# edenartlab/sd-lora-trainer

Hardware: AMD Instinct MI355X
Metric: training images/sec, SDXL 1024px rank-16 LoRA, 1/2/4/8 GPU (job-parallel) (higher is better)
Workload: dtype bf16

## Files before the change

include/sdlt_kernels.h:

```cpp
#ifndef SDLT_KERNELS_H
#define SDLT_KERNELS_H
#include <stdint.h>
#ifdef __cplusplus
extern "C" {
#endif

const char* sdlt_last_error(void);
int sdlt_abi_version(void);
int sdlt_struct_size(int which);

typedef struct sdlt_gemm_batch_item {
  const void* X; const void* W;
  const void* Adown; const void* Bup; void* T_out;
  void* C; void* Ct;
  const float* bias;
  const float* col_scale;
} sdlt_gemm_batch_item;

typedef struct sdlt_gemm_params {
  const void* X; int64_t ldx;
  const void* W; int64_t ldw;
  int32_t M, N, K;
  const void* X2; int64_t ldx2;
  const void* W2; int64_t ldw2;
// ... 411 lines not shown
  float* norm;
  uint8_t* out;
  int32_t n_img, T, P, gh, gw, H, W;
  float alpha;
} sdlt_heatmap_overlay_params;
int sdlt_heatmap_overlay(const sdlt_heatmap_overlay_params* p, void* stream);

int sdlt_token_pool(const void* x, int64_t ldx, int32_t B, int32_t H, int32_t W, int32_t C, const float* gamma, const float* beta, float eps,
                    int32_t f, int32_t mode, void* y, int64_t ldy, int32_t Nkp, void* stream);

int sdlt_tile_blend(const float* tile, int64_t ld, int32_t th, int32_t tw, int32_t C, const float* wy, const float* wx,
                    float* out, int32_t H, int32_t W, int32_t y0, int32_t x0, void* stream);

typedef struct {
  const int32_t* ys; const int32_t* xs;
  const float* wy; const float* wx;
  int32_t n, H, W, th, tw, ty, tx, pad_;
} sdlt_window_params;
int sdlt_window_gather(const sdlt_window_params* p, const void* x_full, void* x_tiles, int64_t ld, const float* tf_full, float* tf_tiles, void* stream);
int sdlt_window_blend(const sdlt_window_params* p, const float* eps_tiles, float* eps_full, void* stream);

int sdlt_add2d(const void* a, int64_t lda, const void* b, int64_t ldb, void* out, int64_t ldo, int32_t M, int32_t C, void* stream);

int sdlt_embed_gather(const void* table, int64_t ld_table, const int64_t* ids, const void* pos, int64_t ld_pos,
                      int32_t B, int32_t T, int32_t Tp, int32_t D, void* out, int64_t ldo, void* stream);
int sdlt_embed_grad(const void* dx, int64_t lddx, const int64_t* ids, const int64_t* train_ids, int32_t n_train,
                    int32_t B, int32_t T, int32_t Tp, int32_t D, float* grad, int32_t accumulate, void* stream);
int sdlt_ti_std_reg(const float* rows, int32_t n, int32_t D, float target_mean, float target_var, float weight,
                    float* grad, float* loss_out, void* stream);

typedef struct sdlt_strip_params {
  const void* X; int64_t ldx;
  const void* W; int64_t ldw;
  const float* bias;
  const void* R; int64_t ldr;
  void* Y; int64_t ldy;
  void* Y2; int64_t ldy2;
  const void* Z; int64_t ldz;
  const float* c1; const float* c2;
  float* stats;
  int32_t B, T, Tp, N, K, act, ln;
  float eps;
  int32_t splitk, cnt_len;
  void* ws; int64_t ws_bytes;
  int32_t* cnt;
  float* P; int64_t ldp;
} sdlt_strip_params;
int sdlt_strip_gemm(const sdlt_strip_params* p, void* stream);

int sdlt_strip_gemm_pair(const sdlt_strip_params* a, const sdlt_strip_params* b, void* stream);
int sdlt_attn_pair_ok(const sdlt_attn_params* a, const sdlt_attn_params* b);
int sdlt_attn_fwd_pair(const sdlt_attn_params* a, const sdlt_attn_params* b, void* stream);
int sdlt_attn_bwd_pair(const sdlt_attn_params* a, const sdlt_attn_params* b, void* stream);
typedef struct sdlt_ln_slabs_params {
  const void* x; int64_t ldx;
  const float* dy32; int64_t lddy32;
  const float* gamma; const float* stats;
  const void* dres; int64_t lddres;
  void* dx; int64_t lddx;
  int32_t nslab, M, C, pad_;
} sdlt_ln_slabs_params;
int sdlt_layernorm_bwd_slabs_pair(const sdlt_ln_slabs_params* a, const sdlt_ln_slabs_params* b, void* stream);

int sdlt_wsk_gemm(const void* X, int64_t ldx, const void* W, int64_t ldw, int32_t M, int32_t N, int32_t K, const float* bias,
                  const void* R, int64_t ldr, void* Y, int64_t ldy, const void* Adown, int64_t ld_adown, const void* Bup, int64_t ld_bup,
                  float lora_scale, void* T_out, int64_t ld_t, int32_t lora_group_k, void* stream);

int sdlt_wsk_gemm_rowdot(const void* X, int64_t ldx, const void* W, int64_t ldw, int32_t M, int32_t N, int32_t K, const float* bias,
                         const void* O, int64_t ldo, void* Y, int64_t ldy, const void* Adown, int64_t ld_adown, const void* Bup, int64_t ld_bup,
                         float lora_scale, void* T_out, int64_t ld_t, int32_t lora_group_k, float* D, int32_t Nq, void* stream);

int sdlt_wsk_pack_weight(const void* W, int64_t ldw, int32_t N, int32_t K, void* Wp, void* stream);

int sdlt_wsk_conv(const void* X, int64_t ldx, const void* W, int64_t ldw, int32_t B, int32_t H, int32_t Wd, int32_t Cin, int32_t N, int32_t flip,
                  const float* bias, const void* rowbias, int64_t ld_rowbias, const void* R, int64_t ldr, void* Y, int64_t ldy,
                  const void* Adown, int64_t ld_adown, const void* Bup, int64_t ld_bup, float lora_scale, void* T_out, int64_t ld_t,
                  const void* zero, void* stream);

int sdlt_wsk_gemm_ln(const void* X, int64_t ldx, const void* W, int64_t ldw, int32_t M, int32_t N, int32_t K, const float* c2,
                     const void* R, int64_t ldr, void* Y, int64_t ldy, const void* Adown, int64_t ld_adown, const void* Bup, int64_t ld_bup,
                     float lora_scale, void* T_out, int64_t ld_t, const float* ln_c1, float* ln_stats, float ln_eps,
                     const float* ln_adapter, void* stream);

typedef struct sdlt_wsk_gemm_params {
  const void* X; int64_t ldx;
  const void* W; int64_t ldw;
  const float* bias;
  const void* R; int64_t ldr;
  void* Y; int64_t ldy;
  const void* Adown; int64_t ld_adown;
  const void* Bup; int64_t ld_bup;
  void* T_out; int64_t ld_t;
  const float* col_scale;
  void* Y0; int64_t ldy0;
  const float* ln_c1; float* ln_stats; const float* ln_adapter;
  void* ln_parts;
  float* dotD;
  const void* pf_next_w;
  int32_t M, N, K;
  int32_t lora_group_k, lora_rp, dot_nq;
  float lora_scale, ln_eps;
  int32_t pf_next_n, pf_next_k, pf_steps, pad_;
} sdlt_wsk_gemm_params;
int sdlt_wsk_gemm_p(const sdlt_wsk_gemm_params* p, void* stream);

int sdlt_wsk_gemm_parts(const void* X, int64_t ldx, const void* W, int64_t ldw, int32_t M, int32_t N, int32_t K, const float* bias,
// ... 28 lines not shown
```

sd-lora-trainer_amd/_lib.py:

```python
import ctypes as C
import os

import torch

_HERE = os.path.dirname(os.path.abspath(__file__))
LIB_PATH = os.environ.get("SDLT_KERNEL_LIB") or os.path.join(_HERE, "libsdlt_kernels.so")

i32, i64, f32, vp = C.c_int32, C.c_int64, C.c_float, C.c_void_p


class GemmParams(C.Structure):
    _fields_ = [
        ("X", vp), ("ldx", i64), ("W", vp), ("ldw", i64),
        ("M", i32), ("N", i32), ("K", i32),
        ("X2", vp), ("ldx2", i64), ("W2", vp), ("ldw2", i64),
        ("K2", i32), ("mode", i32),
        ("Hin", i32), ("Win", i32), ("Cin", i32), ("Hout", i32), ("Wout", i32),
        ("stride", i32), ("ups", i32), ("flip", i32), ("tr", i32),
        ("zero", vp),
        ("Adown", vp), ("ld_adown", i64), ("Bup", vp), ("ld_bup", i64),
        ("T_out", vp), ("ld_t", i64),
        ("lora_R", i32), ("lora_scale", f32), ("alpha", f32),
        ("bias", vp),
        ("rowbias", vp), ("ld_rowbias", i64), ("rows_per_batch", i32),
# ... 222 lines not shown
    "sdlt_groupnorm_fwd": (i32, [C.POINTER(GroupNormParams), vp]),
    "sdlt_groupnorm_bwd": (i32, [C.POINTER(GroupNormParams), vp]),
    "sdlt_layernorm_fwd": (i32, [vp, i64, i32, i32, vp, vp, f32, vp, i64, vp, vp]),
    "sdlt_layernorm_bwd": (i32, [vp, i64, vp, i64, i32, i32, vp, vp, vp, i64, vp, i64, vp]),
    "sdlt_layernorm_bwd_y": (i32, [vp, i64, vp, i64, i32, i32, vp, vp, vp, vp, i64, vp, i64, vp, i64, vp]),
    "sdlt_ln_fold_adapters": (i32, [vp, i32, vp]),
    "sdlt_layernorm_bwd_slabs": (i32, [vp, i64, vp, i64, i32, i32, i32, vp, vp, vp, i64, vp, i64, vp]),
    "sdlt_geglu_fwd": (i32, [vp, i64, i32, i32, vp, i64, vp]),
    "sdlt_geglu_bwd": (i32, [vp, i64, vp, i64, i32, i32, vp, i64, vp]),
    "sdlt_map_bf16": (i32, [i32, vp, vp, vp, i64, vp]),
    "sdlt_timestep_embedding": (i32, [vp, i32, i32, vp, i64, vp]),
    "sdlt_add_noise_nhwc": (i32, [vp, vp, vp, vp, i32, i32, i32, i32, vp, vp, vp]),
    "sdlt_masked_mse_fwd_bwd": (i32, [vp, i64, vp, vp, vp, vp, vp, i32, i32, i32, i32, f32, i32, f32, vp, i32, vp, vp, vp]),
    "sdlt_adamw_fused": (i32, [vp, vp, vp, vp, i64, vp, vp, vp]),
    "sdlt_prodigy_step": (i32, [vp, vp, vp, vp, vp, vp, i64, vp, vp, vp, vp, vp]),
    "sdlt_wgrad_transpose": (i32, [vp, i64, i32, i32, vp, i64, i32, vp, vp]),
    "sdlt_wgrad_im2col_t": (i32, [vp, i64, i32, i32, i32, i32, i32, i32, vp, i64, i32, vp]),
    "sdlt_wgrad_transpose_batch": (i32, [vp, i32, i64, i32, i32, i64, i32, vp]),
    "sdlt_affine_grad_batch": (i32, [vp, i32, i32, i64, i32, i64, i64, i32, i32, i32, f32, i32, vp]),
    "sdlt_wgrad_im2col_t_batch": (i32, [vp, i32, i64, i32, i32, i32, i32, i32, i32, i64, i32, vp]),
    "sdlt_layernorm_affine_grad": (i32, [vp, i64, vp, i64, i32, i32, vp, vp, vp, i32, vp]),
    "sdlt_groupnorm_affine_grad": (i32, [vp, vp, vp, i32, vp]),
    "sdlt_lora_shadow_refresh": (i32, [vp, vp, vp, i32, vp, vp]),
    "sdlt_adamw_shadow_refresh": (i32, [vp, vp, vp, i32, vp, vp, vp, vp, vp, vp]),
    "sdlt_adamw8_shadow_refresh": (i32, [vp, vp, vp, i32, vp, vp, vp, vp, vp, vp, vp, vp]),
    "sdlt_adamw8_flat": (i32, [vp, vp, vp, vp, vp, i64, vp, vp, vp]),
    "sdlt_dora_refresh": (i32, [vp, vp, vp, i32, i32, i32, vp]),
    "sdlt_dora_scale_wt": (i32, [vp, vp, vp, i32, vp]),
    "sdlt_dora_mag_grad": (i32, [vp, vp, vp, i32, vp, vp, i32, vp, vp]),
    "sdlt_lora_merge": (i32, [vp, vp, vp, i32, i32, i32, vp]),
    "sdlt_delta_matmul": (i32, [vp, vp, vp, i32, i32, vp]),
    "sdlt_sampler_step": (i32, [C.POINTER(SamplerParams), vp]),
    "sdlt_sampler_step_img": (i32, [C.POINTER(SamplerImgParams), vp]),
    "sdlt_sampler_step_ms": (i32, [C.POINTER(SamplerMsParams), vp]),
    "sdlt_sampler_step_sde": (i32, [C.POINTER(SamplerSdeParams), vp]),
    "sdlt_sampler_step_dd": (i32, [C.POINTER(SamplerDdParams), vp]),
    "sdlt_sampler_noise": (i32, [vp, i32, i32, i32, vp, vp]),
    "sdlt_guidance": (i32, [C.POINTER(GuidanceParams), vp]),
    "sdlt_resize_planes": (i32, [C.POINTER(ResizeParams), vp]),
    "sdlt_blur_planes": (i32, [vp, vp, vp, i32, i32, i32, vp, i32, i32, vp]),
    "sdlt_freeu_ws_floats": (i64, [i32, i32, i32, i32, i32]),
    "sdlt_freeu": (i32, [vp, i64, vp, i64, vp, i64, vp, i64, i32, i32, i32, i32, i32, f32, f32, i32, vp, vp, vp, i64, vp]),
    "sdlt_heatmap_accum": (i32, [C.POINTER(HeatAccumParams), vp]),
    "sdlt_heatmap_overlay": (i32, [C.POINTER(HeatOverlayParams), vp]),
    "sdlt_token_pool": (i32, [vp, i64, i32, i32, i32, i32, vp, vp, f32, i32, i32, vp, i64, i32, vp]),
    "sdlt_tile_blend": (i32, [vp, i64, i32, i32, i32, vp, vp, vp, i32, i32, i32, i32, vp]),
    "sdlt_window_gather": (i32, [C.POINTER(WindowParams), vp, vp, i64, vp, vp, vp]),
    "sdlt_window_blend": (i32, [C.POINTER(WindowParams), vp, vp, vp]),
    "sdlt_strip_gemm": (i32, [C.POINTER(StripParams), vp]),
    "sdlt_strip_gemm_pair": (i32, [C.POINTER(StripParams), C.POINTER(StripParams), vp]),
    "sdlt_attn_pair_ok": (i32, [C.POINTER(AttnParams), C.POINTER(AttnParams)]),
    "sdlt_attn_fwd_pair": (i32, [C.POINTER(AttnParams), C.POINTER(AttnParams), vp]),
    "sdlt_attn_bwd_pair": (i32, [C.POINTER(AttnParams), C.POINTER(AttnParams), vp]),
    "sdlt_layernorm_bwd_slabs_pair": (i32, [C.POINTER(LnSlabsParams), C.POINTER(LnSlabsParams), vp]),
    "sdlt_wsk_gemm": (i32, [vp, i64, vp, i64, i32, i32, i32, vp, vp, i64, vp, i64, vp, i64, vp, i64, f32, vp, i64, i32, vp]),
    "sdlt_wsk_gemm_rowdot": (i32, [vp, i64, vp, i64, i32, i32, i32, vp, vp, i64, vp, i64, vp, i64, vp, i64, f32, vp, i64, i32, vp, i32, vp]),
    "sdlt_wsk_pack_weight": (i32, [vp, i64, i32, i32, vp, vp]),
    "sdlt_wsk_conv": (i32, [vp, i64, vp, i64, i32, i32, i32, i32, i32, i32, vp, vp, i64, vp, i64, vp, i64, vp, i64, vp, i64, f32, vp, i64, vp, vp]),
    "sdlt_wsk_gemm_parts": (i32, [vp, i64, vp, i64, i32, i32, i32, vp, vp, i64, vp, i64, vp, i64, vp, i64, f32, vp, i64, i32, vp, vp]),
    "sdlt_wsk_gemm_p": (i32, [C.POINTER(WskGemmParams), vp]),
    "sdlt_wsk_gemm_ln": (i32, [vp, i64, vp, i64, i32, i32, i32, vp, vp, i64, vp, i64, vp, i64, vp, i64, f32, vp, i64, vp, vp, f32, vp, vp]),
    "sdlt_token_attention_ws_floats": (i64, [C.POINTER(TaParams)]),
    "sdlt_token_attention_loss": (i32, [C.POINTER(TaParams), vp]),
    "sdlt_sum2x2": (i32, [vp, i32, i32, i32, i32, vp, vp]),
    "sdlt_colsum": (i32, [vp, i64, i32, i32, i32, vp, i64, vp, vp, vp]),
    "sdlt_embed_gather": (i32, [vp, i64, vp, vp, i64, i32, i32, i32, i32, vp, i64, vp]),
    "sdlt_embed_grad": (i32, [vp, i64, vp, vp, i32, i32, i32, i32, i32, vp, i32, vp]),
    "sdlt_ti_std_reg": (i32, [vp, i32, i32, f32, f32, f32, vp, vp, vp]),
}

_lib = None


class KernelLibraryError(RuntimeError):
    pass


def load():
    global _lib
    if _lib is not None:
        return _lib
    if not os.path.exists(LIB_PATH):
        raise KernelLibraryError(
            f"{LIB_PATH} is missing: build it with `python -c 'import __graft_entry__ as g; g.build()'` "
            "(hipcc --offload-arch=gfx950).  There is no CPU / PyTorch fallback for the training step.")
    lib = C.CDLL(LIB_PATH, mode=C.RTLD_GLOBAL)
    for name, (res, args) in SYMBOLS.items():
        try:
            fn = getattr(lib, name)
        except AttributeError as e:
            raise KernelLibraryError(f"{LIB_PATH} does not export {name}") from e
        fn.restype = res
        fn.argtypes = args
    for which, (name, size) in enumerate(struct_sizes()):
        if lib.sdlt_struct_size(which) != size:
            raise KernelLibraryError(f"struct layout mismatch for {name}: C {lib.sdlt_struct_size(which)} vs binding {size}")
    if C.sizeof(ResizeParams) != 48:
        raise KernelLibraryError(f"struct layout mismatch for ResizeParams: header 48 vs binding {C.sizeof(ResizeParams)}")
    for cls, size in ((HeatAccumParams, 152), (HeatOverlayParams, 80), (GemmPlan, 64), (SamplerDdParams, 128), (WindowParams, 64)):
        if C.sizeof(cls) != size:
            raise KernelLibraryError(f"struct layout mismatch for {cls.__name__}: header {size} vs binding {C.sizeof(cls)}")
    _lib = lib
    return lib


def struct_sizes():
# ... 14 lines not shown
```

sd-lora-trainer_amd/clip.py:

```python
import math
import os

import torch

from . import ops as _ops
from .unet import F32, LayerNorm, Linear, StackedLinear, _Module

T_TOKENS = 77
TP = 128


ACT_EPILOGUE = os.environ.get("SDLT_CLIP_ACT_EPI", "1") != "0"


class _Renamed(dict):

    def __init__(self, sd, prefix):
        self.sd, self.prefix = sd, prefix

    def __getitem__(self, k):
        return self.sd[k[len(self.prefix):]]

    def get(self, k, default=None):
        return self.sd.get(k[len(self.prefix):], default)
# ... 50 lines not shown
        rt.ops.attn_bwd(self.q._b["y"], self.k._b["y"], self.v._b["y"], None, None, self._b["O"], self._b["L"], dO,
                        None, self.buf("Dd", B * self.heads * T_TOKENS, dtype=F32), dq, dk, dv, **self._akw(B))
        if self.qkv.has_lora and not self.qkv.kgrouped:
            dn1 = self.q.backward(dq)
            dn1 = self.k.backward(dk, dres=dn1, key="dx2")
            dn1 = self.v.backward(dv, dres=dn1, key="dx3")
        else:
            dn1 = self.qkv.backward(dqkv)
        return self.ln1.backward(dn1, dres=dx1)


FUSED = os.environ.get("SDLT_CLIP_FUSED", "1") != "0"
FUSED_MAXB = int(os.environ.get("SDLT_CLIP_FUSED_MAXB", "4"))


def fused_ok(rt, B, D, F_, arena):
    if not FUSED or arena is not None or not hasattr(rt.ops, "strip_gemm") or B > FUSED_MAXB:
        return False
    return bool(getattr(rt.ops, "STRIP_ANY_SHAPE", False)) or (D % 256 == 0 and F_ % 256 == 0)


class FusedClipLayer(_Module):

    def __init__(self, rt, name, sd, heads, act):
        super().__init__(rt, name)
        dev, dt = rt.device, rt.act
        g = lambda k: sd[name + k].to(dev, F32)
        wq, wk, wv = g(".self_attn.q_proj.weight"), g(".self_attn.k_proj.weight"), g(".self_attn.v_proj.weight")
        wqkv = torch.cat([wq, wk, wv], 0)
        bqkv = torch.cat([g(".self_attn.q_proj.bias"), g(".self_attn.k_proj.bias"), g(".self_attn.v_proj.bias")])
        self.g1, self.be1 = g(".layer_norm1.weight").contiguous(), g(".layer_norm1.bias").contiguous()
        self.g2, self.be2 = g(".layer_norm2.weight").contiguous(), g(".layer_norm2.bias").contiguous()
        self.eps = 1e-5
        fold = rt.ops.fold_layernorm
        self.Wqkv_g, self.qkv_c1, self.qkv_c2 = fold(wqkv, bqkv, self.g1, self.be1, dtype=dt)
        self.Wqkv_t = wqkv.t().to(dt).contiguous()
        wo = g(".self_attn.out_proj.weight")
        self.Wo, self.Wo_t, self.bo = wo.to(dt).contiguous(), wo.t().to(dt).contiguous(), g(".self_attn.out_proj.bias").contiguous()
        w1, w2 = g(".mlp.fc1.weight"), g(".mlp.fc2.weight")
        self.W1_g, self.fc1_c1, self.fc1_c2 = fold(w1, g(".mlp.fc1.bias"), self.g2, self.be2, dtype=dt)
        self.W1_t = w1.t().to(dt).contiguous()
        self.W2, self.W2_t, self.b2 = w2.to(dt).contiguous(), w2.t().to(dt).contiguous(), g(".mlp.fc2.bias").contiguous()
        self.D, self.F, self.heads = wo.shape[0], w1.shape[0], heads
        self.d = self.D // heads
        self.scale = 1.0 / math.sqrt(self.d)
        self.act_kind = "quick_gelu" if act == "quick_gelu" else "gelu"

    def _akw(self, B):
        return dict(B=B, H=self.heads, Nq=T_TOKENS, Nk=T_TOKENS, Nqp=TP, Nkp=TP, d=self.d, scale=self.scale, causal=True)

    def zbuf(self, key, *shape, dtype=None):
        return self.buf(key, *shape, dtype=dtype, zero=True)

    def forward_steps(self, x, B, out=None):
        ops, M, D, F_ = self.rt.ops, B * TP, self.D, self.F
        kw = dict(B=B, T=T_TOKENS, Tp=TP)
        self._x, self._B = x, B
        qkv = ops.strip_gemm(x, self.Wqkv_g, self.zbuf("qkv", M, 3 * D), ln=(self.qkv_c1, self.qkv_c2, self.eps),
                             stats=self.zbuf("st1", M * 2, dtype=F32), **kw)
        yield
        q, k, v = qkv[:, :D], qkv[:, D:2 * D], qkv[:, 2 * D:]
        O, L = self.zbuf("O", M, D), self.zbuf("L", B * self.heads * T_TOKENS, dtype=F32)
        ops.attn_fwd(q, k, v, None, O, L, **self._akw(B))
        yield
        x1 = ops.strip_gemm(O, self.Wo, self.zbuf("x1", M, D), bias=self.bo, residual=x, **kw)
        yield
        a = self.zbuf("a", M, F_)
        ops.strip_gemm(x1, self.W1_g, self.zbuf("y1", M, F_), ln=(self.fc1_c1, self.fc1_c2, self.eps), stats=self.zbuf("st2", M * 2, dtype=F32),
                       act_out=(self.act_kind, a), **kw)
        yield
        y = ops.strip_gemm(a, self.W2, out if out is not None else self.zbuf("x2", M, D), bias=self.b2, residual=x1, **kw)
        yield
        return y

    def forward(self, x, B, out=None):
        return _drain(self.forward_steps(x, B, out))

    def backward_steps(self, dx2):
        ops, B, D, F_ = self.rt.ops, self._B, self.D, self.F
        M = B * TP
        kw = dict(B=B, T=T_TOKENS, Tp=TP)
        b = self._b
        df = ops.strip_gemm(dx2, self.W2_t, self.zbuf("df", M, F_), dact_in=(self.act_kind, b["y1"]), **kw)
        yield
        S2 = ops.strip_partial_splits(D, F_, B)
        dn2 = ops.strip_gemm(df, self.W1_t, None, partial=self.zbuf("dn2_p", S2, M, D, dtype=F32), **kw)
        yield
        dx1 = ops.layernorm_bwd(b["x1"], None, self.zbuf("dx1", M, D), b["st2"], gamma=self.g2, dres=dx2, dy_slabs=dn2)
        yield
        dO = ops.strip_gemm(dx1, self.Wo_t, self.zbuf("dO", M, D), **kw)
        yield
        qkv, dqkv = b["qkv"], self.zbuf("dqkv", M, 3 * D)
        ops.attn_bwd(qkv[:, :D], qkv[:, D:2 * D], qkv[:, 2 * D:], None, None, b["O"], b["L"], dO, None,
                     self.zbuf("Dd", B * self.heads * T_TOKENS, dtype=F32), dqkv[:, :D], dqkv[:, D:2 * D], dqkv[:, 2 * D:], **self._akw(B))
        yield
        S1 = ops.strip_partial_splits(D, 3 * D, B)
        dn1 = ops.strip_gemm(dqkv, self.Wqkv_t, None, partial=self.zbuf("dn1_p", S1, M, D, dtype=F32), **kw)
        yield
        dx = ops.layernorm_bwd(self._x, None, self.zbuf("dx", M, D), b["st1"], gamma=self.g1, dres=dx1, dy_slabs=dn1)
        yield
        return dx

    def backward(self, dx2):
        return _drain(self.backward_steps(dx2))


def _drain(gen):
    while True:
        try:
            next(gen)
        except StopIteration as e:
            return e.value


def _sub(gen, key):
    while True:
        try:
            next(gen)
        except StopIteration as e:
            return e.value
        yield key


class ClipTextEncoder(_Module):

    def __init__(self, rt, name, sd, *, heads, act, mode, with_projection, n_train, arena=None, lora_prefix=""):
        super().__init__(rt, name)
        pre = "text_model." if "text_model.embeddings.token_embedding.weight" in sd else ""
        tab = sd[pre + "embeddings.token_embedding.weight"]
        self.V, self.D = tab.shape
        self.n_train = n_train
        self.table = tab.to(rt.device, rt.act).contiguous()
        self.pos = sd[pre + "embeddings.position_embedding.weight"].to(rt.device, rt.act).contiguous()
        nl = 0
        while f"{pre}encoder.layers.{nl}.layer_norm1.weight" in sd:
            nl += 1
        self.mode, self.with_projection = mode, with_projection
        self.n_run = nl if (mode == "last" or with_projection) else nl - 1
        self.n_hidden = nl if mode == "last" else nl - 1
        mlp = sd[f"{pre}encoder.layers.0.mlp.fc1.weight"].shape[0] if nl else 0
        self.fused = nl > 0 and fused_ok(rt, rt.B, self.D, mlp, arena)
        if self.fused:
            self.layers = [FusedClipLayer(rt, f"{pre}encoder.layers.{i}", sd, heads, act) for i in range(self.n_run)]
        else:
            self.layers = [ClipLayer(rt, f"{pre}encoder.layers.{i}", sd, heads, act, arena, lora_prefix) for i in range(self.n_run)]
        self.final_ln = LayerNorm(rt, pre + "final_layer_norm", sd) if (mode == "last" or with_projection) else None
        self.proj = Linear(rt, "text_projection", sd) if with_projection else None
# ... 64 lines not shown
```

sd-lora-trainer_amd/ops.py:

```python
import collections
import ctypes as C
import math
import os
import weakref

import torch

from . import _lib

BF16 = torch.bfloat16
F32 = torch.float32


def _stream():
    return C.c_void_p(torch.cuda.current_stream().cuda_stream)


def _p(t):
    return C.c_void_p(t.data_ptr()) if t is not None else C.c_void_p(0)


def _ld(t):
    assert t.dim() == 2 and t.stride(1) == 1, f"need a 2-D row-major view, got {tuple(t.shape)} strides {t.stride()}"
    return t.stride(0)
# ... 468 lines not shown
        self.pending = []
        self.launches = 0

    def take(self):
        rec, self.pending = self.pending, []
        return rec

    def launch(self, recs):
        lib, st = _lib.load(), _stream()
        if len(recs) == 2 and recs[0][0] == recs[1][0] and _pair_ok(lib, recs[0], recs[1]):
            kind = recs[0][0]
            _lib.check(getattr(lib, _PAIR_FN[kind])(C.byref(recs[0][1]), C.byref(recs[1][1]), st), _PAIR_FN[kind])
            self.launches += 1
            return
        for kind, p, _ in recs:
            _launch_single(lib, kind, p, st)
            self.launches += 1

    def flush(self):
        self.launch(self.take())


def run_paired(gens, prefer):
    vals, keys, pend, done = [None, None], [None, None], [None, None], [False, False]
    with pairing() as pq:
        while True:
            for i in (0, 1):
                if not done[i] and pend[i] is None:
                    try:
                        keys[i] = next(gens[i])
                    except StopIteration as e:
                        vals[i], done[i] = e.value, True
                    rec = pq.take()
                    if len(rec) > 1 or (done[i] and rec):
                        pq.launch(rec)
                        raise AssertionError("run_paired: a chain issued a pairable op without yielding")
                    pend[i] = rec[0] if rec else None
            if pend[0] is not None and pend[1] is not None:
                if keys[0] == keys[1]:
                    pq.launch([pend[0], pend[1]])
                    pend = [None, None]
                else:
                    i = 0 if prefer(keys[0], keys[1]) == keys[0] else 1
                    pq.launch([pend[i]])
                    pend[i] = None
            elif pend[0] is not None or pend[1] is not None:
                i = 0 if pend[0] is not None else 1
                pq.launch([pend[i]])
                pend[i] = None
            elif done[0] and done[1]:
                return vals


_PAIR_FN = {"strip": "sdlt_strip_gemm_pair", "attn_fwd": "sdlt_attn_fwd_pair", "attn_bwd": "sdlt_attn_bwd_pair", "ln_slabs": "sdlt_layernorm_bwd_slabs_pair"}
_pair_queue = None


class pairing:
    def __enter__(self):
        global _pair_queue
        assert _pair_queue is None
        _pair_queue = _PairQueue()
        return _pair_queue

    def __exit__(self, *exc):
        global _pair_queue
        q, _pair_queue = _pair_queue, None
        if exc[0] is None:
            q.flush()
        return False


def _pair_ok(lib, a, b):
    kind, pa, pb = a[0], a[1], b[1]
    if kind == "strip":
        wide = lambda n: n >= STRIP_WIDE_MIN and n % 32 == 0
        return bool(pa.ln) == bool(pb.ln) and wide(pa.N) == wide(pb.N) and not (pa.splitk > 1 and not pa.P) and not (pb.splitk > 1 and not pb.P)
    if kind in ("attn_fwd", "attn_bwd"):
        return bool(lib.sdlt_attn_pair_ok(C.byref(pa), C.byref(pb)))
    return True


def _launch_single(lib, kind, p, st):
    if kind == "strip":
        _lib.check(lib.sdlt_strip_gemm(C.byref(p), st), "sdlt_strip_gemm")
    elif kind == "attn_fwd":
        _lib.check(lib.sdlt_attn_fwd(C.byref(p), st), "sdlt_attn_fwd")
    elif kind == "attn_bwd":
        _lib.check(lib.sdlt_attn_bwd(C.byref(p), st), "sdlt_attn_bwd")
    else:
        _lib.check(lib.sdlt_layernorm_bwd_slabs(p.x, p.ldx, p.dy32, p.lddy32, p.nslab, p.M, p.C, p.gamma, p.stats, p.dres, p.lddres, p.dx, p.lddx, st),
                   "sdlt_layernorm_bwd_slabs")


def _issue(kind, p, keep=None):
    if _pair_queue is not None:
        _pair_queue.pending.append((kind, p, keep))
    else:
        _launch_single(_lib.load(), kind, p, _stream())


def strip_gemm(X, W, out, *, B, T, Tp, bias=None, residual=None, act_out=None, dact_in=None, ln=None, stats=None, splitk=None, partial=None):
    lib = _lib.load()
    p = _lib.StripParams()
    _chk2(X), _chk2(W)
    N, K = W.shape
    assert X.shape[0] == B * Tp and X.shape[1] == K, (X.shape, W.shape)
    p.X, p.ldx, p.W, p.ldw = _p(X), _ld(X), _p(W), _ld(W)
    p.B, p.T, p.Tp, p.N, p.K = B, T, Tp, N, K
    if partial is not None:
        assert out is None and bias is None and residual is None and act_out is None and dact_in is None and ln is None
        assert partial.is_cuda and partial.dtype == F32 and partial.is_contiguous() and tuple(partial.shape[1:]) == (B * Tp, N)
        p.P, p.ldp, p.splitk = _p(partial), N, partial.shape[0]
        _issue("strip", p)
        return partial
    _chk2(out)
    assert tuple(out.shape) == (B * Tp, N), (out.shape, W.shape)
    p.Y, p.ldy = _p(out), _ld(out)
    if ln is not None:
        c1, c2, eps = ln
        _chk2(c1, F32), _chk2(c2, F32)
        assert c1.numel() == N and c2.numel() == N and bias is None, "with ln the bias is part of c2"
        p.ln, p.c1, p.c2, p.eps = 1, _p(c1), _p(c2), float(eps)
        if stats is not None:
            _chk2(stats, F32)
            assert stats.numel() >= B * Tp * 2
            p.stats = _p(stats)
    elif bias is not None:
        _chk2(bias, F32)
        assert bias.numel() == N
        p.bias = _p(bias)
    if residual is not None:
        _chk2(residual)
        assert tuple(residual.shape) == (B * Tp, N)
        p.R, p.ldr = _p(residual), _ld(residual)
    if act_out is not None or dact_in is not None:
        assert not (act_out is not None and dact_in is not None)
        kind, t = act_out if act_out is not None else dact_in
        _chk2(t)
        assert tuple(t.shape) == (B * Tp, N) and kind in ("gelu", "quick_gelu")
        p.act = 1 if kind == "quick_gelu" else 2
        if act_out is not None:
# ... 135 lines not shown
        if self.Rp > 64:
            _lib.check(lib.sdlt_lora_grad_wide(_p(self.descs_dev), _p(self.block_desc_dev), self.n_blocks, self.Rp, self.mfma, _stream()),
                       "sdlt_lora_grad_wide")
            return
        _lib.check(lib.sdlt_lora_grad_grouped(_p(self.descs_dev), _p(self.block_desc_dev), self.n_blocks, self.Rp, self.mfma, _stream()),
                   "sdlt_lora_grad_grouped")


def _attn_params(Q, K, V, *, B, H, Nq, Nk, Nqp, Nkp, d, scale, causal=False):
    p = _lib.AttnParams()
    for t in (Q, K, V):
        _chk2(t)
    p.Q, p.ldq, p.K, p.ldk, p.V, p.ldv = _p(Q), _ld(Q), _p(K), _ld(K), _p(V), _ld(V)
    p.B, p.H, p.Nq, p.Nk, p.Nqp, p.Nkp, p.d = B, H, Nq, Nk, Nqp, Nkp, d
    p.scale, p.qsplit, p.causal = float(scale), 1, int(causal)
    return p


def attn_fwd(Q, K, V, Vt, O, L, *, B, H, Nq, Nk, Nqp, Nkp, d, scale, causal=False, zero_D=None):
    lib = _lib.load()
    p = _attn_params(Q, K, V, B=B, H=H, Nq=Nq, Nk=Nk, Nqp=Nqp, Nkp=Nkp, d=d, scale=scale, causal=causal)
    _chk2(O), _chk2(L, F32)
    p.O, p.ldo, p.L = _p(O), _ld(O), _p(L)
    if zero_D is not None:
        _chk2(zero_D, F32)
        assert zero_D.is_contiguous() and zero_D.numel() >= B * H * Nq
        p.D = _p(zero_D)
    _issue("attn_fwd", p)
    return O


def attn_bwd(Q, K, V, Kt, Qt, O, L, dO, dOt, D, dQ, dK, dV, *, B, H, Nq, Nk, Nqp, Nkp, d, scale, causal=False,
             qsplit=1, dK32=None, dV32=None, accumulate_dq=False, accumulate_dk=False, defer_splitsum=False, d_ready=False):
    lib = _lib.load()
    p = _attn_params(Q, K, V, B=B, H=H, Nq=Nq, Nk=Nk, Nqp=Nqp, Nkp=Nkp, d=d, scale=scale, causal=causal)
    p.defer_splitsum = int(defer_splitsum)
    p.d_ready = int(d_ready)
    for t in (O, dO, dQ, dK, dV):
        _chk2(t)
    _chk2(L, F32), _chk2(D, F32)
    p.O, p.ldo, p.L, p.dO, p.lddo, p.D = _p(O), _ld(O), _p(L), _p(dO), _ld(dO), _p(D)
    p.dQ, p.lddq, p.dK, p.lddk, p.dV, p.lddv = _p(dQ), _ld(dQ), _p(dK), _ld(dK), _p(dV), _ld(dV)
    p.qsplit = qsplit
    p.accumulate_dq, p.accumulate_dk = int(accumulate_dq), int(accumulate_dk)
    if qsplit > 1:
        _chk2(dK32, F32), _chk2(dV32, F32)
        p.dK32, p.dV32, p.ld32 = _p(dK32), _p(dV32), _ld(dK32)
        code = lib.sdlt_attn_route(C.byref(p), 1)
        if code >= 0 and _lib.attn_route_decode(code)["route"] in ("BWD_CROSS", "BWD_CROSS_ROLES"):
            assert dK32.shape[0] >= qsplit * B * Nkp and dV32.shape[0] >= qsplit * B * Nkp, "dK32/dV32 must hold qsplit slabs"
    _issue("attn_bwd", p)


class SplitsumPlan:

    def __init__(self, items, device):
        arr = (_lib.SplitsumDesc * len(items))()
        counts = []
        for d, it in zip(arr, items):
            s0, s1, o0, o1 = it["dK32"], it["dV32"], it["dK"], it["dV"]
            _chk2(s0, F32), _chk2(s1, F32), _chk2(o0), _chk2(o1)
            Cw = o0.shape[1]
            assert Cw % 4 == 0 and _ld(s0) == _ld(s1) and s0.shape[0] >= it["nsplit"] * it["B"] * it["Nkp"]
            d.s0, d.s1, d.ld32, d.out0, d.ldo0, d.out1, d.ldo1 = _p(s0), _p(s1), _ld(s0), _p(o0), _ld(o0), _p(o1), _ld(o1)
            d.nsplit, d.B, d.Nk, d.Nkp, d.C, d.acc0 = it["nsplit"], it["B"], it["Nk"], it["Nkp"], Cw, int(bool(it.get("acc0")))
            d.nblocks = max(1, min(64, (it["B"] * it["Nkp"] * Cw // 2 + 255) // 256))
            counts.append(d.nblocks)
        self.keep = items
        self.descs_dev = _to_dev(arr, device)
        self.n_blocks, self.bd, self.bf = _block_table(counts, device)

    def run(self):
        _lib.check(_lib.load().sdlt_attn_splitsum_batch(_p(self.descs_dev), _p(self.bd), _p(self.bf), self.n_blocks, _stream()), "sdlt_attn_splitsum_batch")


_GN_WS = {}


def gn_workspace(device):
    owner = _ws_owner if _ws_owner is not None else _gn_owner
    key = (device, ("owner", owner) if owner is not None else torch.cuda.current_stream(device).cuda_stream)
    ws = _GN_WS.get(key)
    if ws is None:
        ws = (torch.empty(1 << 20, dtype=F32, device=device), torch.zeros(256, dtype=torch.int32, device=device))
        _GN_WS[key] = ws
    return ws


def _gn_params(x1, x2, B, HW, gamma, beta, eps, silu, stats):
    p = _lib.GroupNormParams()
    ws, cnt = gn_workspace(x1.device)
    p.ws, p.ws_floats, p.cnt, p.cnt_len = _p(ws), ws.numel(), _p(cnt), cnt.numel()
    _chk2(x1), _chk2(gamma, F32), _chk2(beta, F32), _chk2(stats, F32)
    C1 = x1.shape[1]
    Ctot = C1 + (x2.shape[1] if x2 is not None else 0)
    assert gamma.numel() == Ctot and x1.shape[0] == B * HW and stats.numel() >= B * 64
    p.x1, p.ldx1, p.C1 = _p(x1), _ld(x1), C1
    if x2 is not None:
        _chk2(x2)
        p.x2, p.ldx2 = _p(x2), _ld(x2)
    p.B, p.HW, p.C = B, HW, Ctot
    p.gamma, p.beta, p.eps, p.silu, p.stats = _p(gamma), _p(beta), float(eps), int(silu), _p(stats)
    return p


def groupnorm_fwd(x1, x2, y, stats, *, B, HW, gamma, beta, eps, silu, stats_zeroed=False):
# ... 880 lines not shown
```

Before: 24.61.

## Add single-block causal attention kernels for CLIP text encoder

Adds dedicated HIP forward and backward attention kernels for the short causal text sequences (at most 80 tokens, head dim 64). Each block handles one head and one batch entirely in LDS with MFMA and transpose reads, and the backward computes dQ, dK and dV in one launch without split-sum or a separate D pass. The CLIP layers route to these kernels by default, replacing the general flash-attention path, with paired launch variants for the pair queue. The text encoder is a small part of SDXL training cost, so any gain is limited, and the new specialised code carries correctness risk.

Result: no change. 24.67 (median of 6 runs) (+0.3%).

```diff
diff --git a/include/sdlt_kernels.h b/include/sdlt_kernels.h
--- a/include/sdlt_kernels.h
+++ b/include/sdlt_kernels.h
@@ -487,6 +487,10 @@
 int sdlt_attn_pair_ok(const sdlt_attn_params* a, const sdlt_attn_params* b);
 int sdlt_attn_fwd_pair(const sdlt_attn_params* a, const sdlt_attn_params* b, void* stream);
 int sdlt_attn_bwd_pair(const sdlt_attn_params* a, const sdlt_attn_params* b, void* stream);
+int sdlt_text_attn_fwd(const sdlt_attn_params* p, void* stream);
+int sdlt_text_attn_bwd(const sdlt_attn_params* p, void* stream);
+int sdlt_text_attn_fwd_pair(const sdlt_attn_params* a, const sdlt_attn_params* b, void* stream);
+int sdlt_text_attn_bwd_pair(const sdlt_attn_params* a, const sdlt_attn_params* b, void* stream);
 typedef struct sdlt_ln_slabs_params {
   const void* x; int64_t ldx;
   const float* dy32; int64_t lddy32;
diff --git a/sd-lora-trainer_amd/_lib.py b/sd-lora-trainer_amd/_lib.py
--- a/sd-lora-trainer_amd/_lib.py
+++ b/sd-lora-trainer_amd/_lib.py
@@ -298,6 +298,10 @@
     "sdlt_attn_pair_ok": (i32, [C.POINTER(AttnParams), C.POINTER(AttnParams)]),
     "sdlt_attn_fwd_pair": (i32, [C.POINTER(AttnParams), C.POINTER(AttnParams), vp]),
     "sdlt_attn_bwd_pair": (i32, [C.POINTER(AttnParams), C.POINTER(AttnParams), vp]),
+    "sdlt_text_attn_fwd": (i32, [C.POINTER(AttnParams), vp]),
+    "sdlt_text_attn_bwd": (i32, [C.POINTER(AttnParams), vp]),
+    "sdlt_text_attn_fwd_pair": (i32, [C.POINTER(AttnParams), C.POINTER(AttnParams), vp]),
+    "sdlt_text_attn_bwd_pair": (i32, [C.POINTER(AttnParams), C.POINTER(AttnParams), vp]),
     "sdlt_layernorm_bwd_slabs_pair": (i32, [C.POINTER(LnSlabsParams), C.POINTER(LnSlabsParams), vp]),
     "sdlt_wsk_gemm": (i32, [vp, i64, vp, i64, i32, i32, i32, vp, vp, i64, vp, i64, vp, i64, vp, i64, f32, vp, i64, i32, vp]),
     "sdlt_wsk_gemm_rowdot": (i32, [vp, i64, vp, i64, i32, i32, i32, vp, vp, i64, vp, i64, vp, i64, vp, i64, f32, vp, i64, i32, vp, i32, vp]),
diff --git a/sd-lora-trainer_amd/clip.py b/sd-lora-trainer_amd/clip.py
--- a/sd-lora-trainer_amd/clip.py
+++ b/sd-lora-trainer_amd/clip.py
@@ -126,6 +126,10 @@
     def zbuf(self, key, *shape, dtype=None):
         return self.buf(key, *shape, dtype=dtype, zero=True)
 
+    def _text_attn(self, B):
+        ok = getattr(self.rt.ops, "text_attn_ok", None)
+        return ok is not None and ok(**self._akw(B))
+
     def forward_steps(self, x, B, out=None):
         ops, M, D, F_ = self.rt.ops, B * TP, self.D, self.F
         kw = dict(B=B, T=T_TOKENS, Tp=TP)
@@ -135,7 +139,10 @@
         yield
         q, k, v = qkv[:, :D], qkv[:, D:2 * D], qkv[:, 2 * D:]
         O, L = self.zbuf("O", M, D), self.zbuf("L", B * self.heads * T_TOKENS, dtype=F32)
-        ops.attn_fwd(q, k, v, None, O, L, **self._akw(B))
+        if self._text_attn(B):
+            ops.text_attn_fwd(q, k, v, O, L, **self._akw(B))
+        else:
+            ops.attn_fwd(q, k, v, None, O, L, **self._akw(B))
         yield
         x1 = ops.strip_gemm(O, self.Wo, self.zbuf("x1", M, D), bias=self.bo, residual=x, **kw)
         yield
@@ -165,8 +172,11 @@
         dO = ops.strip_gemm(dx1, self.Wo_t, self.zbuf("dO", M, D), **kw)
         yield
         qkv, dqkv = b["qkv"], self.zbuf("dqkv", M, 3 * D)
-        ops.attn_bwd(qkv[:, :D], qkv[:, D:2 * D], qkv[:, 2 * D:], None, None, b["O"], b["L"], dO, None,
-                     self.zbuf("Dd", B * self.heads * T_TOKENS, dtype=F32), dqkv[:, :D], dqkv[:, D:2 * D], dqkv[:, 2 * D:], **self._akw(B))
+        if self._text_attn(B):
+            ops.text_attn_bwd(qkv[:, :D], qkv[:, D:2 * D], qkv[:, 2 * D:], b["O"], b["L"], dO, dqkv[:, :D], dqkv[:, D:2 * D], dqkv[:, 2 * D:], **self._akw(B))
+        else:
+            ops.attn_bwd(qkv[:, :D], qkv[:, D:2 * D], qkv[:, 2 * D:], None, None, b["O"], b["L"], dO, None,
+                         self.zbuf("Dd", B * self.heads * T_TOKENS, dtype=F32), dqkv[:, :D], dqkv[:, D:2 * D], dqkv[:, 2 * D:], **self._akw(B))
         yield
         S1 = ops.strip_partial_splits(D, 3 * D, B)
         dn1 = ops.strip_gemm(dqkv, self.Wqkv_t, None, partial=self.zbuf("dn1_p", S1, M, D, dtype=F32), **kw)
diff --git a/sd-lora-trainer_amd/csrc/textattn.hip b/sd-lora-trainer_amd/csrc/textattn.hip
--- /dev/null
+++ b/sd-lora-trainer_amd/csrc/textattn.hip
@@ -0,0 +1,351 @@
+#include "common.h"
+#include "../../include/sdlt_kernels.h"
+
+namespace {
+
+constexpr float LOG2E = 1.4426950408889634f;
+constexpr int TW = 80;
+constexpr int TR = 96;
+constexpr int NSTR = 128;
+constexpr int TILE = TR * NSTR;
+constexpr int PSTR = 2 * TR + 16;
+constexpr int NT = 320;
+constexpr int SMEM_FWD = 2 * TILE, SMEM_BWD = 4 * TILE + 2 * TR * PSTR;
+
+__device__ __forceinline__ bf16x8 pack8(const float* a, const float* b) {
+  union { uint4 u; bf16x8 v; } c;
+  c.u.x = pack2bf(a[0], a[1]); c.u.y = pack2bf(a[2], a[3]);
+  c.u.z = pack2bf(b[0], b[1]); c.u.w = pack2bf(b[2], b[3]);
+  return c.v;
+}
+__device__ __forceinline__ bf16x8 ld_frag_global(const bf16_t* p, bool ok) {
+  union { uint4 u; bf16x8 v; } c;
+  c.u = ok ? *(const uint4*)p : make_uint4(0, 0, 0, 0);
+  return c.v;
+}
+__device__ __forceinline__ int prow(int i, int half) { return ((i >> 2) << 3) + half * 4 + (i & 3); }
+__device__ __forceinline__ int row_sw(int row) { return (((row >> 1) & 1) << 1) | (((row >> 3) & 1) << 2); }
+__device__ __forceinline__ bf16x8 lds_tr_frag(const char* p, int stride) {
+  typedef __attribute__((address_space(3))) bf16x4* lds_ptr;
+  bf16x4 lo = __builtin_amdgcn_ds_read_tr16_b64_v4bf16((lds_ptr)p);
+  bf16x4 hi = __builtin_amdgcn_ds_read_tr16_b64_v4bf16((lds_ptr)(p + 4 * stride));
+  return __builtin_shufflevector(lo, hi, 0, 1, 2, 3, 4, 5, 6, 7);
+}
+__device__ __forceinline__ bf16x8 lds_row_frag(const char* tile, int row, int kk, int g) {
+  return *(const bf16x8*)(tile + row * NSTR + (((kk * 4 + g) ^ row_sw(row)) << 4));
+}
+
+struct TileRegs { uint4 r[3]; };
+__device__ __forceinline__ void gload_tile(TileRegs& t, const bf16_t* src, int64_t ld, int64_t row0, int T, int hc) {
+#pragma unroll
+  for (int j = 0; j < 3; ++j) {
+    const int c = threadIdx.x + NT * j, row = c >> 3, ch = c & 7;
+    t.r[j] = row < T ? *(const uint4*)(src + (row0 + row) * ld + hc + ch * 8) : make_uint4(0, 0, 0, 0);
+  }
+}
+__device__ __forceinline__ void sstore_tile(const TileRegs& t, char* dst) {
+#pragma unroll
+  for (int j = 0; j < 3; ++j) {
+    const int c = threadIdx.x + NT * j, row = c >> 3, ch = c & 7;
+    if (c < TR * 8) *(uint4*)(dst + row * NSTR + ((ch ^ row_sw(row)) << 4)) = t.r[j];
+  }
+}
+__device__ __forceinline__ void store4(bf16_t* dst, const f32x4 v, float f) {
+  uint2 w;
+  w.x = pack2bf(v[0] * f, v[1] * f);
+  w.y = pack2bf(v[2] * f, v[3] * f);
+  *(uint2*)dst = w;
+}
+
+__device__ __forceinline__ void text_fwd_body(const sdlt_attn_params& p, char* smem, const int h, const int b) {
+  const int T = p.Nq, hc = h * 64;
+  const int lane = threadIdx.x & 63, wave = __builtin_amdgcn_readfirstlane(threadIdx.x >> 6), g = lane >> 4, i = lane & 15;
+  const int q = wave * 16 + i;
+  const int64_t row0 = (int64_t)b * p.Nqp;
+  char* Ks = smem;
+  char* Vs = smem + TILE;
+  TileRegs kr, vr;
+  gload_tile(kr, (const bf16_t*)p.K, p.ldk, row0, T, hc);
+  gload_tile(vr, (const bf16_t*)p.V, p.ldv, row0, T, hc);
+  bf16x8 qf[2];
+#pragma unroll
+  for (int kk = 0; kk < 2; ++kk) qf[kk] = ld_frag_global((const bf16_t*)p.Q + (row0 + q) * p.ldq + hc + kk * 32 + g * 8, q < T);
+  sstore_tile(kr, Ks);
+  sstore_tile(vr, Vs);
+  __syncthreads();
+  if (wave * 16 >= T) return;
+  const int nkb = (wave + 2) >> 1;
+  const float sl2 = p.scale * LOG2E;
+  f32x4 s[6];
+#pragma unroll
+  for (int kf = 0; kf < 6; ++kf) {
+    s[kf] = (f32x4){0.f, 0.f, 0.f, 0.f};
+    if ((kf >> 1) < nkb) {
+      const int krow = (kf >> 1) * 32 + prow(i, kf & 1);
+#pragma unroll
+      for (int kk = 0; kk < 2; ++kk) s[kf] = __builtin_amdgcn_mfma_f32_16x16x32_bf16(lds_row_frag(Ks, krow, kk, g), qf[kk], s[kf], 0, 0, 0);
+    }
+#pragma unroll
+    for (int r = 0; r < 4; ++r) {
+      const int key = (kf >> 1) * 32 + g * 8 + (kf & 1) * 4 + r;
+      if (key >= T || key > q) s[kf][r] = -1e30f;
+    }
+  }
+  float tmax = -1e30f;
+#pragma unroll
+  for (int kf = 0; kf < 6; ++kf)
+#pragma unroll
+    for (int r = 0; r < 4; ++r) tmax = fmaxf(tmax, s[kf][r]);
+  tmax = fmaxf(tmax, __shfl_xor(tmax, 16, 64));
+  tmax = fmaxf(tmax, __shfl_xor(tmax, 32, 64));
+  const float m = tmax * sl2;
+  float lsum = 0.f;
+#pragma unroll
+  for (int kf = 0; kf < 6; ++kf)
+#pragma unroll
+    for (int r = 0; r < 4; ++r) {
+      const float pv = __builtin_amdgcn_exp2f(__builtin_fmaf(s[kf][r], sl2, -m));
+      s[kf][r] = pv;
+      lsum += pv;
+    }
+  lsum += __shfl_xor(lsum, 16, 64);
+  lsum += __shfl_xor(lsum, 32, 64);
+  f32x4 o[4];
+#pragma unroll
+  for (int df = 0; df < 4; ++df) o[df] = (f32x4){0.f, 0.f, 0.f, 0.f};
+  const int troff = (8 * g + (i >> 2)) * NSTR + (i & 3) * 8;
+  const int tsw = row_sw(8 * g + (i >> 2)) >> 1;
+#pragma unroll
+  for (int kb = 0; kb < 3; ++kb) {
+    if (kb < nkb) {
+      float a4[4] = {s[2 * kb][0], s[2 * kb][1], s[2 * kb][2], s[2 * kb][3]};
+      float b4[4] = {s[2 * kb + 1][0], s[2 * kb + 1][1], s[2 * kb + 1][2], s[2 * kb + 1][3]};
+      const bf16x8 pf = pack8(a4, b4);
+#pragma unroll
+      for (int df = 0; df < 4; ++df) {
+        const bf16x8 vf = lds_tr_frag(Vs + troff + kb * 32 * NSTR + ((df ^ tsw) << 5), NSTR);
+        o[df] = __builtin_amdgcn_mfma_f32_16x16x32_bf16(vf, pf, o[df], 0, 0, 0);
+      }
+    }
+  }
+  if (q < T) {
+    const float inv = 1.f / lsum;
+    if (g == 0) p.L[((int64_t)b * p.H + h) * T + q] = (m + log2f(lsum)) / LOG2E;
+#pragma unroll
+    for (int df = 0; df < 4; ++df) store4((bf16_t*)p.O + (row0 + q) * p.ldo + hc + df * 16 + g * 4, o[df], inv);
+  }
+}
+
+__global__ __launch_bounds__(NT) void attn_text_fwd_kernel(const sdlt_attn_params p) {
+  extern __shared__ __attribute__((aligned(16))) char smem[];
+  text_fwd_body(p, smem, blockIdx.x, blockIdx.y);
+}
+__global__ __launch_bounds__(NT) void attn_text_fwd_pair_kernel(const sdlt_attn_params p0, const sdlt_attn_params p1) {
+  extern __shared__ __attribute__((aligned(16))) char smem[];
+  const int x = blockIdx.x, y = blockIdx.y;
+  if (x < p0.H) {
+    if (y < p0.B) text_fwd_body(p0, smem, x, y);
+  } else if (y < p1.B) {
+    text_fwd_body(p1, smem, x - p0.H, y);
+  }
+}
+
+__device__ __forceinline__ void text_bwd_body(const sdlt_attn_params& p, char* smem, const int h, const int b) {
+  const int T = p.Nq, hc = h * 64;
+  const int lane = threadIdx.x & 63, wave = __builtin_amdgcn_readfirstlane(threadIdx.x >> 6), g = lane >> 4, i = lane & 15;
+  const int q = wave * 16 + i;
+  const bool qok = q < T;
+  const int64_t row0 = (int64_t)b * p.Nqp;
+  char* Ks = smem;
+  char* Vs = Ks + TILE;
+  char* Qs = Vs + TILE;
+  char* Gs = Qs + TILE;
+  char* Ps = Gs + TILE;
+  char* Ss = Ps + TR * PSTR;
+  {
+    TileRegs kr, vr, qr, gr;
+    gload_tile(kr, (const bf16_t*)p.K, p.ldk, row0, T, hc);
+    gload_tile(vr, (const bf16_t*)p.V, p.ldv, row0, T, hc);
+    gload_tile(qr, (const bf16_t*)p.Q, p.ldq, row0, T, hc);
+    gload_tile(gr, (const bf16_t*)p.dO, p.lddo, row0, T, hc);
+    sstore_tile(kr, Ks);
+    sstore_tile(vr, Vs);
+    sstore_tile(qr, Qs);
+    sstore_tile(gr, Gs);
+  }
+  if (threadIdx.x < (TR - TW) * PSTR / 16) {
+    *(uint4*)(Ps + TW * PSTR + threadIdx.x * 16) = make_uint4(0, 0, 0, 0);
+    *(uint4*)(Ss + TW * PSTR + threadIdx.x * 16) = make_uint4(0, 0, 0, 0);
+  }
+  const int qlim = min(p.Nqp, (T + 63) & ~63), klim = p.Nkp;
+  for (int c = TW * 16 + threadIdx.x; c < klim * 16; c += NT) {
+    const int row = c >> 4, col = hc + (c & 15) * 4;
+    if (row < qlim) *(uint2*)((bf16_t*)p.dQ + (row0 + row) * p.lddq + col) = make_uint2(0, 0);
+    *(uint2*)((bf16_t*)p.dK + (row0 + row) * p.lddk + col) = make_uint2(0, 0);
+    *(uint2*)((bf16_t*)p.dV + (row0 + row) * p.lddv + col) = make_uint2(0, 0);
+  }
+  bf16x8 qf[2], gf[2];
+  float Dq = 0.f;
+#pragma unroll
+  for (int kk = 0; kk < 2; ++kk) {
+    const int col = hc + kk * 32 + g * 8;
+    qf[kk] = ld_frag_global((const bf16_t*)p.Q + (row0 + q) * p.ldq + col, qok);
+    gf[kk] = ld_frag_global((const bf16_t*)p.dO + (row0 + q) * p.lddo + col, qok);
+    const bf16x8 of = ld_frag_global((const bf16_t*)p.O + (row0 + q) * p.ldo + col, qok);
+#pragma unroll
+    for (int j = 0; j < 8; ++j) Dq += (float)gf[kk][j] * (float)of[j];
+  }
+  Dq += __shfl_xor(Dq, 16, 64);
+  Dq += __shfl_xor(Dq, 32, 64);
+  const float Lq = qok ? p.L[((int64_t)b * p.H + h) * T + q] * LOG2E : 0.f;
+  if (p.D && g == 0 && qok) p.D[((int64_t)b * p.H + h) * T + q] = Dq;
+  const float sl2 = p.scale * LOG2E;
+  const int troff = (8 * g + (i >> 2)) * NSTR + (i & 3) * 8;
+  const int tsw = row_sw(8 * g + (i >> 2)) >> 1;
+  __syncthreads();
+
+  {
+    const int nkb = (wave + 2) >> 1;
+    f32x4 dq[4];
+#pragma unroll
+    for (int df = 0; df < 4; ++df) dq[df] = (f32x4){0.f, 0.f, 0.f, 0.f};
+#pragma unroll
+    for (int kb = 0; kb < 3; ++kb) {
+      if (kb < nkb) {
+        f32x4 s[2], dp[2];
+#pragma unroll
+        for (int hf = 0; hf < 2; ++hf) {
+          s[hf] = (f32x4){0.f, 0.f, 0.f, 0.f};
+          dp[hf] = (f32x4){0.f, 0.f, 0.f, 0.f};
+          const int krow = kb * 32 + prow(i, hf);
+#pragma unroll
+          for (int kk = 0; kk < 2; ++kk) {
+            s[hf] = __builtin_amdgcn_mfma_f32_16x16x32_bf16(lds_row_frag(Ks, krow, kk, g), qf[kk], s[hf], 0, 0, 0);
+            dp[hf] = __builtin_amdgcn_mfma_f32_16x16x32_bf16(lds_row_frag(Vs, krow, kk, g), gf[kk], dp[hf], 0, 0, 0);
+          }
+#pragma unroll
+          for (int r = 0; r < 4; ++r) {
+            const int key = kb * 32 + g * 8 + hf * 4 + r;
+            const bool ok = qok && key < T && key <= q;
+            const float pv = ok ? __builtin_amdgcn_exp2f(__builtin_fmaf(s[hf][r], sl2, -Lq)) : 0.f;
+            s[hf][r] = pv;
+            dp[hf][r] = pv * (dp[hf][r] - Dq);
+          }
+        }
+        float a4[4] = {s[0][0], s[0][1], s[0][2], s[0][3]};
+        float b4[4] = {s[1][0], s[1][1], s[1][2], s[1][3]};
+        float c4[4] = {dp[0][0], dp[0][1], dp[0][2], dp[0][3]};
+        float e4[4] = {dp[1][0], dp[1][1], dp[1][2], dp[1][3]};
+        const bf16x8 pf = pack8(a4, b4), dsf = pack8(c4, e4);
+        *(bf16x8*)(Ps + q * PSTR + (kb * 32 + g * 8) * 2) = pf;
+        *(bf16x8*)(Ss + q * PSTR + (kb * 32 + g * 8) * 2) = dsf;
+#pragma unroll
+        for (int df = 0; df < 4; ++df) {
+          const bf16x8 ktf = lds_tr_frag(Ks + troff + kb * 32 * NSTR + ((df ^ tsw) << 5), NSTR);
+          dq[df] = __builtin_amdgcn_mfma_f32_16x16x32_bf16(ktf, dsf, dq[df], 0, 0, 0);
+        }
+      }
+    }
+    if (q < qlim) {
+#pragma unroll
+      for (int df = 0; df < 4; ++df) store4((bf16_t*)p.dQ + (row0 + q) * p.lddq + hc + df * 16 + g * 4, dq[df], p.scale);
+    }
+  }
+  __syncthreads();
+
+  {
+    f32x4 dk[4], dv[4];
+#pragma unroll
+    for (int df = 0; df < 4; ++df) {
+      dk[df] = (f32x4){0.f, 0.f, 0.f, 0.f};
+      dv[df] = (f32x4){0.f, 0.f, 0.f, 0.f};
+    }
+    const int qb_end = (T + 31) >> 5;
+#pragma unroll
+    for (int qb = 0; qb < 3; ++qb) {
+      if (qb >= (wave >> 1) && qb < qb_end) {
+        const int poff = (qb * 32 + 8 * g + (i >> 2)) * PSTR + (wave * 16 + 4 * (i & 3)) * 2;
+        const bf16x8 pf = lds_tr_frag(Ps + poff, PSTR), dsf = lds_tr_frag(Ss + poff, PSTR);
+#pragma unroll
+        for (int df = 0; df < 4; ++df) {
+          const bf16x8 gtf = lds_tr_frag(Gs + troff + qb * 32 * NSTR + ((df ^ tsw) << 5), NSTR);
+          dv[df] = __builtin_amdgcn_mfma_f32_16x16x32_bf16(gtf, pf, dv[df], 0, 0, 0);
+          const bf16x8 qtf = lds_tr_frag(Qs + troff + qb * 32 * NSTR + ((df ^ tsw) << 5), NSTR);
+          dk[df] = __builtin_amdgcn_mfma_f32_16x16x32_bf16(qtf, dsf, dk[df], 0, 0, 0);
+        }
+      }
+    }
+    const int key = wave * 16 + i;
+    if (key < klim) {
+#pragma unroll
+      for (int df = 0; df < 4; ++df) {
+        store4((bf16_t*)p.dK + (row0 + key) * p.lddk + hc + df * 16 + g * 4, dk[df], p.scale);
+        store4((bf16_t*)p.dV + (row0 + key) * p.lddv + hc + df * 16 + g * 4, dv[df], 1.f);
+      }
+    }
+  }
+}
+
+__global__ __launch_bounds__(NT) void attn_text_bwd_kernel(const sdlt_attn_params p) {
+  extern __shared__ __attribute__((aligned(16))) char smem[];
+  text_bwd_body(p, smem, blockIdx.x, blockIdx.y);
+}
+__global__ __launch_bounds__(NT) void attn_text_bwd_pair_kernel(const sdlt_attn_params p0, const sdlt_attn_params p1) {
+  extern __shared__ __attribute__((aligned(16))) char smem[];
+  const int x = blockIdx.x, y = blockIdx.y;
+  if (x < p0.H) {
+    if (y < p0.B) text_bwd_body(p0, smem, x, y);
+  } else if (y < p1.B) {
+    text_bwd_body(p1, smem, x - p0.H, y);
+  }
+}
+
+int text_check(const sdlt_attn_params& p, bool backward, const char* fn) {
+  if (p.B <= 0 || p.H <= 0 || p.B > 65535 || p.d != 64 || !p.causal || p.Nq <= 0 || p.Nq > TW || p.Nk != p.Nq || p.Nqp < p.Nq || p.Nkp != p.Nqp || (p.Nqp % 8) || p.qsplit != 1 ||
+      p.accumulate_dq || p.accumulate_dk)
+    SDLT_FAIL(SDLT_ERR_UNSUPPORTED, "%s: B=%d H=%d Nq=%d Nk=%d Nqp=%d Nkp=%d d=%d causal=%d qsplit=%d (causal, d == 64, Nq == Nk <= 80, Nqp == Nkp a multiple of 8 only)", fn, p.B,
+              p.H, p.Nq, p.Nk, p.Nqp, p.Nkp, p.d, p.causal, p.qsplit);
+  if (!p.Q || !p.K || !p.V || !p.O || !p.L || (backward && (!p.dO || !p.dQ || !p.dK || !p.dV))) SDLT_FAIL(SDLT_ERR_SHAPE, "%s: missing operand", fn);
+  if ((p.ldq % 8) || (p.ldk % 8) || (p.ldv % 8) || (((uintptr_t)p.Q | (uintptr_t)p.K | (uintptr_t)p.V) % 16)) SDLT_FAIL(SDLT_ERR_ALIGN, "%s: Q / K / V need 16-byte rows", fn);
+  if (!backward) {
+    if ((p.ldo % 4) || ((uintptr_t)p.O % 8)) SDLT_FAIL(SDLT_ERR_ALIGN, "%s: O needs 8-byte rows", fn);
+    return SDLT_OK;
+  }
+  if ((p.ldo % 8) || (p.lddo % 8) || (((uintptr_t)p.O | (uintptr_t)p.dO) % 16)) SDLT_FAIL(SDLT_ERR_ALIGN, "%s: O / dO need 16-byte rows", fn);
+  if ((p.lddq % 4) || (p.lddk % 4) || (p.lddv % 4) || (((uintptr_t)p.dQ | (uintptr_t)p.dK | (uintptr_t)p.dV) % 8)) SDLT_FAIL(SDLT_ERR_ALIGN, "%s: dQ / dK / dV need 8-byte rows", fn);
+  return SDLT_OK;
+}
+
+template <typename... A>
+int text_launch(void (*k)(A...), dim3 grid, int smem, void* stream, const char* fn, const A&... args) {
+  if (sdlt_raise_smem((const void*)k, smem)) SDLT_FAIL(SDLT_ERR_LAUNCH, "%s: LDS attribute", fn);
+  hipLaunchKernelGGL(k, grid, dim3(NT), smem, (hipStream_t)stream, args...);
+  const hipError_t e = hipGetLastError();
+  if (e != hipSuccess) SDLT_FAIL(SDLT_ERR_LAUNCH, "%s: %s", fn, hipGetErrorString(e));
+  return SDLT_OK;
+}
+
+}
+
+extern "C" int sdlt_text_attn_fwd(const sdlt_attn_params* p, void* stream) {
+  const int rc = text_check(*p, false, "sdlt_text_attn_fwd");
+  return rc ? rc : text_launch(attn_text_fwd_kernel, dim3(p->H, p->B), SMEM_FWD, stream, "sdlt_text_attn_fwd", *p);
+}
+extern "C" int sdlt_text_attn_bwd(const sdlt_attn_params* p, void* stream) {
+  const int rc = text_check(*p, true, "sdlt_text_attn_bwd");
+  return rc ? rc : text_launch(attn_text_bwd_kernel, dim3(p->H, p->B), SMEM_BWD, stream, "sdlt_text_attn_bwd", *p);
+}
+extern "C" int sdlt_text_attn_fwd_pair(const sdlt_attn_params* a, const sdlt_attn_params* b, void* stream) {
+  for (const sdlt_attn_params* q : {a, b}) {
+    const int rc = text_check(*q, false, "sdlt_text_attn_fwd_pair");
+    if (rc) return rc;
+  }
+  return text_launch(attn_text_fwd_pair_kernel, dim3(a->H + b->H, a->B > b->B ? a->B : b->B), SMEM_FWD, stream, "sdlt_text_attn_fwd_pair", *a, *b);
+}
+extern "C" int sdlt_text_attn_bwd_pair(const sdlt_attn_params* a, const sdlt_attn_params* b, void* stream) {
+  for (const sdlt_attn_params* q : {a, b}) {
+    const int rc = text_check(*q, true, "sdlt_text_attn_bwd_pair");
+    if (rc) return rc;
+  }
+  return text_launch(attn_text_bwd_pair_kernel, dim3(a->H + b->H, a->B > b->B ? a->B : b->B), SMEM_BWD, stream, "sdlt_text_attn_bwd_pair", *a, *b);
+}
diff --git a/sd-lora-trainer_amd/ops.py b/sd-lora-trainer_amd/ops.py
--- a/sd-lora-trainer_amd/ops.py
+++ b/sd-lora-trainer_amd/ops.py
@@ -544,7 +544,9 @@
                 return vals
 
 
-_PAIR_FN = {"strip": "sdlt_strip_gemm_pair", "attn_fwd": "sdlt_attn_fwd_pair", "attn_bwd": "sdlt_attn_bwd_pair", "ln_slabs": "sdlt_layernorm_bwd_slabs_pair"}
+_PAIR_FN = {"strip": "sdlt_strip_gemm_pair", "attn_fwd": "sdlt_attn_fwd_pair", "attn_bwd": "sdlt_attn_bwd_pair", "ln_slabs": "sdlt_layernorm_bwd_slabs_pair",
+            "text_attn_fwd": "sdlt_text_attn_fwd_pair", "text_attn_bwd": "sdlt_text_attn_bwd_pair"}
+_SINGLE_FN = {"attn_fwd": "sdlt_attn_fwd", "attn_bwd": "sdlt_attn_bwd", "text_attn_fwd": "sdlt_text_attn_fwd", "text_attn_bwd": "sdlt_text_attn_bwd"}
 _pair_queue = None
 
 
@@ -576,10 +578,8 @@
 def _launch_single(lib, kind, p, st):
     if kind == "strip":
         _lib.check(lib.sdlt_strip_gemm(C.byref(p), st), "sdlt_strip_gemm")
-    elif kind == "attn_fwd":
-        _lib.check(lib.sdlt_attn_fwd(C.byref(p), st), "sdlt_attn_fwd")
-    elif kind == "attn_bwd":
-        _lib.check(lib.sdlt_attn_bwd(C.byref(p), st), "sdlt_attn_bwd")
+    elif kind in _SINGLE_FN:
+        _lib.check(getattr(lib, _SINGLE_FN[kind])(C.byref(p), st), _SINGLE_FN[kind])
     else:
         _lib.check(lib.sdlt_layernorm_bwd_slabs(p.x, p.ldx, p.dy32, p.lddy32, p.nslab, p.M, p.C, p.gamma, p.stats, p.dres, p.lddres, p.dx, p.lddx, st),
                    "sdlt_layernorm_bwd_slabs")
@@ -821,6 +821,35 @@
     _issue("attn_bwd", p)
 
 
+TEXT_ATTN = os.environ.get("SDLT_TEXT_ATTN", "1") != "0"
+
+
+def text_attn_ok(*, Nq, Nk, Nqp, Nkp, d, causal, **_):
+    return TEXT_ATTN and bool(causal) and d == 64 and Nq == Nk <= 80 and Nqp == Nkp and Nqp % 8 == 0
+
+
+def text_attn_fwd(Q, K, V, O, L, *, B, H, Nq, Nk, Nqp, Nkp, d, scale, causal=True):
+    p = _attn_params(Q, K, V, B=B, H=H, Nq=Nq, Nk=Nk, Nqp=Nqp, Nkp=Nkp, d=d, scale=scale, causal=causal)
+    _chk2(O), _chk2(L, F32)
+    p.O, p.ldo, p.L = _p(O), _ld(O), _p(L)
+    _issue("text_attn_fwd", p)
+    return O
+
+
+def text_attn_bwd(Q, K, V, O, L, dO, dQ, dK, dV, *, B, H, Nq, Nk, Nqp, Nkp, d, scale, causal=True, D=None):
+    p = _attn_params(Q, K, V, B=B, H=H, Nq=Nq, Nk=Nk, Nqp=Nqp, Nkp=Nkp, d=d, scale=scale, causal=causal)
+    for t in (O, dO, dQ, dK, dV):
+        _chk2(t)
+    _chk2(L, F32)
+    p.O, p.ldo, p.L, p.dO, p.lddo = _p(O), _ld(O), _p(L), _p(dO), _ld(dO)
+    p.dQ, p.lddq, p.dK, p.lddk, p.dV, p.lddv = _p(dQ), _ld(dQ), _p(dK), _ld(dK), _p(dV), _ld(dV)
+    if D is not None:
+        _chk2(D, F32)
+        assert D.is_contiguous() and D.numel() >= B * H * Nq
+        p.D = _p(D)
+    _issue("text_attn_bwd", p)
+
+
 class SplitsumPlan:
 
     def __init__(self, items, device):
```
